# jxbi1010/VLA-Touch

Measured on AMD Instinct MI355X. Metric: refined action chunks/sec (RDT-1B chunk + DINOv2 x2 + pi_I), higher is better.
Workload: dtype bf16 model, 16-bit activations in IEEE fp16 (RDT-1B --rdt-compute f16, DINOv2 tower; same width and MFMA rate as bf16)

## Files before the change

### vla-touch_amd/csrc/vt_api.hip

```cpp
#include <string.h>
#include "vt_common.h"
#include "vt_kernels.h"
#include "vt_host.h"
#include "vt_gemm_route.h"
#include "vt_prof.h"
#include "vt_unet_int.h"
#include "../../include/vlatouch.h"

VtProfState g_vt_prof;

extern "C" {

const char* vt_last_error(void) { return vt_errbuf(); }
int vt_version(void) { return 100; }

int vt_gemm(const void* params, vt_stream_t stream) {
  if (!params) return vt_fail(VT_ERR_ARG, "vt_gemm: null params");
  const int r = vt_gemm_launch(*reinterpret_cast<const VtGemmParams*>(params), (hipStream_t)stream);
  if (r) vt_fail(r, "vt_gemm: rejected (alignment: K, lda, ldw multiples of 8 bf16 / 4 fp32; conv: cin likewise) or launch failure");
  return r;
}
int vt_gemm_route_of(const void* params) {
  if (!params) return VT_ROUTE_BAD_ARG;
  return vt_gemm_route(*reinterpret_cast<const VtGemmParams*>(params));
}
int vt_gemm_route_split(const void* params, int* head_route, int* tail_route) {
  if (!params || !head_route || !tail_route) return vt_fail(VT_ERR_ARG, "vt_gemm_route_split: null argument");
  const VtGemmParams& p = *reinterpret_cast<const VtGemmParams*>(params);
  if (vt_gemm_route(p) != VT_GEMM_ROWSPLIT) return vt_fail(VT_ERR_ARG, "vt_gemm_route_split: the block does not route to VT_ROUTE_ROWSPLIT");
  VtGemmParams head, tail;
  *head_route = vt_gemm_rowsplit(p, head, tail);
  *tail_route = vt_gemm_route(tail);
  return VT_OK;
}
int vt_tune(int knob, int value) {
  if (knob == 1 && (value == 0 || value == 4 || value == 8)) { vt_gemm_pw_tune(value); return VT_OK; }
  if (knob == 2 || knob == 8) { vt_gemm_route_tune(knob, value); return VT_OK; }
  if (knob == 4) { vt_gemm_pws_tune(value); return VT_OK; }
  if (knob == 6) { vt_attn_kvt_tune(value); return VT_OK; }
  if (knob == 7) { vt_unet_fused_tune(value); return VT_OK; }
  if (knob == 9 && (value == 0 || value == 1 || value == 3 || value == 6)) { vt_attn16g_tune(value); return VT_OK; }
  return vt_fail(VT_ERR_ARG, "vt_tune: unknown knob %d / value %d", knob, value);
}
int vt_prof_enable(int on) {
  g_vt_prof.on = on != 0;
  g_vt_prof.mode = on > 1 ? on : 1;
  if (on) { g_vt_prof.used = 0; g_vt_prof.flops = 0.0; g_vt_prof.bytes = 0.0; }
  return VT_OK;
}
int vt_prof_collect(double* total_ms, double* flops, double* bytes, long* launches) {
  double ms = 0.0;
  for (int i = 0; i < g_vt_prof.used; ++i) {
    float t = 0.f;
    if (hipEventElapsedTime(&t, g_vt_prof.ev[2 * i], g_vt_prof.ev[2 * i + 1]) != hipSuccess) return VT_ERR_LAUNCH;
    ms += t;
  }
  if (total_ms) *total_ms = ms;
  if (flops) *flops = g_vt_prof.flops;
  if (bytes) *bytes = g_vt_prof.bytes;
  if (launches) *launches = g_vt_prof.used;
  return VT_OK;
}
int vt_attention(const void* params, vt_stream_t stream) {
  if (!params) return vt_fail(VT_ERR_ARG, "vt_attention: null params");
  const int r = vt_attn_launch(*reinterpret_cast<const VtAttnParams*>(params), (hipStream_t)stream);
  if (r) vt_fail(r, "vt_attention: bad strides/sizes or launch failure");
  return r;
}
int vt_attention_kvt(const void* params, vt_stream_t stream) {
  if (!params) return vt_fail(VT_ERR_ARG, "vt_attention_kvt: null params");
  const int r = vt_attn_kvt_launch(*reinterpret_cast<const VtAttnKvtParams*>(params), (hipStream_t)stream);
  if (r) vt_fail(r, "vt_attention_kvt: bad sizes / strides (T * 64 >= B * Nk, q_rs % 8), parts without part_ws or > 16, or launch failure");
  return r;
}
size_t vt_attention_kvt_part_bytes(int B, int H, int Nq, int parts) { return vt_attn_kvt_part_bytes(B, H, Nq, parts); }
int vt_retile_kv(const void* K, const void* V, long ld, void* KV, int M, int T, int H, vt_stream_t stream) {
  if (!K || !V || !KV || M < 1 || H < 1) return vt_fail(VT_ERR_ARG, "vt_retile_kv: null source / destination or empty shape");
  const int r = vt_k_retile_kv(K, V, ld, KV, M, T, H, (hipStream_t)stream);
  if (r) vt_fail(r, "vt_retile_kv: T * 64 < M, ld % 8 or launch failure");
  return r;
}
int vt_groupnorm(const void* params, vt_stream_t stream) {
  if (!params) return vt_fail(VT_ERR_ARG, "vt_groupnorm: null params");
  const int r = vt_k_groupnorm(*reinterpret_cast<const VtGnParams*>(params), (hipStream_t)stream);
  if (r) vt_fail(r, "vt_groupnorm: unsupported group size or launch failure");
  return r;
}
int vt_rownorm(const void* x, int xdt, long ldx, void* y, int ydt, long ldy, const float* w, const float* b, int rows, int D, float eps,
               int mode, vt_stream_t stream) {
  const int r = vt_k_rownorm(x, xdt, ldx, y, ydt, ldy, w, b, rows, D, eps, mode, (hipStream_t)stream);
  if (r) vt_fail(r, "vt_rownorm: D must be a multiple of 4 and <= 2048");
  return r;
}
int vt_headnorm(void* x, int dt, long tok_stride, int heads, long tokens, const float* w, float eps, int mode, vt_stream_t stream) {
  return vt_k_headnorm(x, dt, tok_stride, heads, tokens, w, eps, mode, (hipStream_t)stream);
}
int vt_action_normalize(const float* in, float* out, const float* mins, const float* maxs, long n, int dim, float padding_factor,
                        int denormalize, vt_stream_t stream) {
  if (!in || !out || !mins || !maxs || n < 0 || dim < 1) return vt_fail(VT_ERR_ARG, "vt_action_normalize: bad argument");
  if (n == 0) return VT_OK;
  return vt_k_actnorm(in, out, mins, maxs, n, dim, padding_factor, denormalize, (hipStream_t)stream);
}

}

static_assert(VT_ROUTE_UNSUPPORTED == VT_GEMM_UNSUPPORTED && VT_ROUTE_BAD_ARG == VT_GEMM_BAD_ARG && VT_ROUTE_REG == VT_GEMM_REG && VT_ROUTE_F32R == VT_GEMM_F32R &&
              VT_ROUTE_GLDS == VT_GEMM_GLDS && VT_ROUTE_PP == VT_GEMM_PP && VT_ROUTE_PT == VT_GEMM_PT && VT_ROUTE_PPK == VT_GEMM_PPK && VT_ROUTE_PW == VT_GEMM_PW &&
              VT_ROUTE_PWS == VT_GEMM_PWS && VT_ROUTE_ROWSPLIT == VT_GEMM_ROWSPLIT, "include/vlatouch.h route codes = enum VtGemmRoute");

namespace {
template <typename T>
__global__ void mfma_selftest_kernel(float* err) {
  const int lane = threadIdx.x, g = lane >> 4, l15 = lane & 15;
  Frag<T> a, b;
  float av[8], bv[8];
  for (int j = 0; j < 8; ++j) {
    const int k = g * 8 + j;
    av[j] = (k == l15) ? 1.f : 0.f;
    bv[j] = (float)(l15 * 100 + k);
  }
  if constexpr (sizeof(T) == 2) {
    for (int j = 0; j < 8; ++j) { a.v[j] = (short)f2bf(av[j]); b.v[j] = (short)f2bf(bv[j]); }
  } else {
    for (int j = 0; j < 8; ++j) { a.v[j] = av[j]; b.v[j] = bv[j]; }
  }
  float4_t acc = {0.f, 0.f, 0.f, 0.f};
  mma16(acc, a, b);
  float e = 0.f;
  for (int r = 0; r < 4; ++r) {
    const int row = g * 4 + r, col = l15;
    float expect = (float)(col * 100 + row);
    if constexpr (sizeof(T) == 2) expect = bf2f(f2bf(expect));
    e = fmaxf(e, fabsf(acc[r] - expect));
  }
  e = wave_max(e);
  if (lane == 0) *err = e;
}
}

extern "C" int vt_selftest_mfma(float* out_err, vt_stream_t stream) {
  if (!out_err) return vt_fail(VT_ERR_ARG, "vt_selftest_mfma: null");
  hipLaunchKernelGGL((mfma_selftest_kernel<bf16_t>), dim3(1), dim3(64), 0, (hipStream_t)stream, out_err);
  hipLaunchKernelGGL((mfma_selftest_kernel<float>), dim3(1), dim3(64), 0, (hipStream_t)stream, out_err + 1);
  return vt_check_launch();
}

namespace {
__device__ __forceinline__ void philox_round(uint32_t (&c)[4], const uint32_t k0, const uint32_t k1) {
  const uint64_t p0 = (uint64_t)0xD2511F53u * c[0], p1 = (uint64_t)0xCD9E8D57u * c[2];
  const uint32_t n0 = (uint32_t)(p1 >> 32) ^ c[1] ^ k0, n1 = (uint32_t)p1, n2 = (uint32_t)(p0 >> 32) ^ c[3] ^ k1, n3 = (uint32_t)p0;
  c[0] = n0; c[1] = n1; c[2] = n2; c[3] = n3;
}
__device__ __forceinline__ void philox4x32_10(uint32_t (&c)[4], uint32_t k0, uint32_t k1) {
#pragma unroll
  for (int r = 0; r < 10; ++r) { philox_round(c, k0, k1); k0 += 0x9E3779B9u; k1 += 0xBB67AE85u; }
}
__global__ void randn_kernel(float* __restrict__ out, const long n, const unsigned long long* __restrict__ state, const int round_bf16) {
  const long q = (long)blockIdx.x * blockDim.x + threadIdx.x;
  if (q * 4 >= n) return;
  const unsigned long long key = state[0], ctr = state[1] + (unsigned long long)q;
  uint32_t c[4] = {(uint32_t)ctr, (uint32_t)(ctr >> 32), 0u, 0u};
  philox4x32_10(c, (uint32_t)key, (uint32_t)(key >> 32));
  float v[4];
#pragma unroll
  for (int h = 0; h < 2; ++h) {
    const float u1 = ((float)(c[2 * h] >> 8) + 0.5f) * (1.0f / 16777216.0f);
    const float u2 = ((float)(c[2 * h + 1] >> 8) + 0.5f) * (1.0f / 16777216.0f);
    const float r = sqrtf(-2.0f * __logf(u1));
    float sn, cs;
    __sincosf(6.283185307179586f * u2, &sn, &cs);
    v[2 * h] = r * cs; v[2 * h + 1] = r * sn;
  }
#pragma unroll
  for (int j = 0; j < 4; ++j) {
    if (round_bf16) v[j] = bf2f(f2bf(v[j]));
    if (q * 4 + j < n) out[q * 4 + j] = v[j];
  }
}
__global__ void randn_advance_kernel(unsigned long long* state, const unsigned long long by) { state[1] += by; }
template <typename TI>
__global__ void slice_cast_kernel(const TI* __restrict__ in, float* __restrict__ out, int B, int Tin, int Din, int T, int Dd) {
  const long i = (long)blockIdx.x * blockDim.x + threadIdx.x;
  if (i >= (long)B * T * Dd) return;
  const int d = (int)(i % Dd);
  const long r = i / Dd;
  const int t = (int)(r % T), b = (int)(r / T);
  out[i] = Elem<TI>::to_f(in[((long)b * Tin + t) * Din + d]);
}
}

extern "C" int vt_randn(float* out, long n, void* state, int round_bf16, vt_stream_t stream) {
  if (!out || !state || n < 0) return vt_fail(VT_ERR_ARG, "vt_randn: null argument");
  if (n == 0) return VT_OK;
  const long quads = (n + 3) / 4;
  hipLaunchKernelGGL(randn_kernel, dim3((unsigned)((quads + 255) / 256)), dim3(256), 0, (hipStream_t)stream, out, n, (const unsigned long long*)state, round_bf16);
  hipLaunchKernelGGL(randn_advance_kernel, dim3(1), dim3(1), 0, (hipStream_t)stream, (unsigned long long*)state, (unsigned long long)quads);
  return vt_check_launch();
}
extern "C" int vt_slice_cast(const void* in, int idt, float* out, int B, int Tin, int Din, int T, int Dd, vt_stream_t stream) {
  if (!in || !out || B < 1 || T < 1 || Dd < 1 || T > Tin || Dd > Din) return vt_fail(VT_ERR_ARG, "vt_slice_cast: bad shape");
  const long n = (long)B * T * Dd;
  const dim3 grid((unsigned)((n + 255) / 256));
  if (idt == VT_BF16) hipLaunchKernelGGL((slice_cast_kernel<bf16_t>), grid, dim3(256), 0, (hipStream_t)stream, (const bf16_t*)in, out, B, Tin, Din, T, Dd);
  else if (idt == VT_F32) hipLaunchKernelGGL((slice_cast_kernel<float>), grid, dim3(256), 0, (hipStream_t)stream, (const float*)in, out, B, Tin, Din, T, Dd);
  else return vt_fail(VT_ERR_UNSUPPORTED, "vt_slice_cast: bf16 or fp32 input");
  return vt_check_launch();
}

extern "C" int vt_cast(const void* in, int idt, long ldi, void* out, int odt, long ldo, int rows, int cols, vt_stream_t stream) {
  if (!in || !out || rows < 1 || cols < 1) return vt_fail(VT_ERR_ARG, "vt_cast: bad argument");
  const int r = vt_k_act_copy(in, idt, ldi, out, odt, ldo, rows, cols, VT_ACT_NONE, (hipStream_t)stream);
  if (r) vt_fail(r, "vt_cast: unsupported dtype pair");
  return r;
}
```

### vla-touch_amd/csrc/vt_gemm_pw.hip

```cpp
#include "vt_common.h"
#include "vt_gemm_route.h"
#include "vt_gemm_epilogue.h"
#include "vt_prof.h"
#include "vt_host.h"
#include "vt_kernels.h"
#include "../../include/vlatouch.h"

namespace {

constexpr int BM = 160, BN = 128, BK = 64;
constexpr int TMW = BM / 32;
constexpr int A_TILE = BM * 128;
constexpr int OPS = BM / 8 / 4 + 4;

template <typename T16, typename TC, int NB, int FUSE = 0>
__global__ __launch_bounds__(256, 1) void gemm_pw_kernel(const VtGemmParams p, const int tiles_n, const int tiles_per_group, const int total_tiles, const int GM) {
  constexpr int SMEM = NB * A_TILE > BM * BN * 4 ? NB * A_TILE : BM * BN * 4;
  __shared__ __attribute__((aligned(16))) char smem[SMEM];
  const int tid = threadIdx.x, lane = tid & 63;
  const int wave = __builtin_amdgcn_readfirstlane(tid >> 6);
  const int l31 = lane & 31, hk = lane >> 5;

  int bid = blockIdx.x;
  if ((total_tiles & 7) == 0) bid = (bid & 7) * (total_tiles >> 3) + (bid >> 3);
  const int grp = bid / tiles_per_group;
  const int t_in = bid - grp * tiles_per_group;
  const int tiles_m = tiles_per_group / tiles_n;
  const int sr = t_in / (GM * tiles_n);
  const int gmr = min(GM, tiles_m - sr * GM);
  const int r_in = t_in - sr * GM * tiles_n;
  const int tn = r_in / gmr, tm = sr * GM + (r_in - tn * gmr);
  const int m0 = tm * BM, n0 = tn * BN;

  const uint16_t* A = reinterpret_cast<const uint16_t*>(p.A) + (long)grp * p.a_gs;
  const int nk = p.K / BK;

  const __amdgpu_buffer_rsrc_t rsA = __builtin_amdgcn_make_buffer_rsrc((void*)(A + (long)m0 * p.lda), 0, 0x7fffffff, 0x00020000);
  int asrc[5];
#pragma unroll
  for (int e = 0; e < 5; ++e) {
    const int r = (wave + 4 * e) * 8 + (lane >> 3);
    const int c = (lane & 7) ^ ((r >> 1) & 7);
    asrc[e] = (int)(((long)(min(m0 + r, p.M - 1) - m0) * p.lda + c * 8) * 2);
  }
  const char* wbase = reinterpret_cast<const char*>(p.Wp) + ((long)grp * p.w_gs) * 2 + ((long)(n0 / 32 + wave) * (p.K / 16)) * 1024;
  wbase = VT_UNIFORM_PTR(wbase);
  const unsigned wvoff = lane * 16;

  int4_t wb[NB][4];
  auto issue = [&](const int kt, auto bc) {
    constexpr int b = decltype(bc)::value;
#pragma unroll
    for (int e = 0; e < 5; ++e)
      __builtin_amdgcn_raw_ptr_buffer_load_lds(rsA, (lds_void*)(smem + b * A_TILE + (wave + 4 * e) * 1024), 16, asrc[e], kt * (BK * 2), 0, 0);
    const char* sb = wbase + (long)kt * 4096;
    wload<0, true>(wb[b][0], wvoff, sb);
    wload<1024, false>(wb[b][1], wvoff, sb);
    wload<2048, false>(wb[b][2], wvoff, sb);
    wload<3072, false>(wb[b][3], wvoff, sb);
  };

  const int xr = (l31 >> 1) & 7;
  int foff[4];
#pragma unroll
  for (int s = 0; s < 4; ++s) foff[s] = l31 * 128 + (((s * 2 + hk) ^ xr) * 16);
  auto frags = [&](int4_t (&f)[TMW], const int b, const int s) {
#pragma unroll
    for (int j = 0; j < TMW; ++j) f[j] = *reinterpret_cast<const int4_t*>(smem + b * A_TILE + j * 4096 + foff[s]);
  };

  float16_t acc[TMW];
#pragma unroll
  for (int j = 0; j < TMW; ++j)
#pragma unroll
    for (int r = 0; r < 16; ++r) acc[j][r] = 0.f;

  static_for<NB - 1>([&](auto bc) { if (decltype(bc)::value < nk) issue(decltype(bc)::value, bc); });
  vt_wait_vm<(NB - 3) * OPS>(wb[0]);
  vt_wait_vm<(NB - 3) * OPS>(wb[1]);
  __builtin_amdgcn_sched_barrier(0);
  __builtin_amdgcn_s_barrier();
  __builtin_amdgcn_sched_barrier(0);
  int4_t af[2][TMW];
  frags(af[0], 0, 0);

  constexpr int RSV = FUSE == 2 ? (BM * 16 + 255) / 256 : 1;
  float4 rsv[RSV];
  auto sub = [&](const int t, auto uc, auto tailc) {
    constexpr int U = decltype(uc)::value;
    constexpr bool TAIL = decltype(tailc)::value;
    if constexpr (!TAIL || U == 0) issue(t + NB - 1, std::integral_constant<int, (U + NB - 1) % NB>{});
    if constexpr (FUSE == 2 && TAIL && U == NB - 2) {
      const int h2 = p.rs_n >> 1, nq = BM * h2;
#pragma unroll
      for (int i = 0; i < RSV; ++i) {
        const int q = tid + 256 * i;
        const int row = q / h2, c = q - row * h2;
        rsv[i] = q < nq ? *reinterpret_cast<const float4*>(p.rs_part + ((long)min(m0 + row, p.M - 1) * p.rs_n + 2 * c) * 2) : make_float4(0.f, 0.f, 0.f, 0.f);
      }
    }
#pragma unroll
    for (int s = 0; s < 4; ++s) {
      if (s < 3) frags(af[(s + 1) & 1], U, s + 1);
      else if (!TAIL || U < NB - 1) frags(af[0], (U + 1) % NB, 0);
#pragma unroll
      for (int j = 0; j < TMW; ++j) acc[j] = mma32<T16>(wb[U][s], af[s & 1][j], acc[j]);
    }
#pragma unroll
    for (int i = 0; i < 4 * TMW; ++i) {
      __builtin_amdgcn_sched_group_barrier(0x008, 1, 0);
      __builtin_amdgcn_sched_group_barrier(0x100, 1, 0);
    }
    if constexpr (!TAIL) vt_wait_vm<(NB - 3) * OPS>(wb[(U + 2) % NB]);
    else if constexpr (U + 2 < NB) vt_wait_vm<(NB - 3 - U > 0 ? NB - 3 - U : 0) * OPS>(wb[(U + 2) % NB]);
    __builtin_amdgcn_sched_barrier(0);
    __builtin_amdgcn_s_barrier();
    __builtin_amdgcn_sched_barrier(0);
  };
  int t = 0;
  for (; t + NB < nk; t += NB) static_for<NB>([&](auto uc) { sub(t + decltype(uc)::value, uc, std::false_type{}); });
  static_for<NB>([&](auto uc) { sub(t + decltype(uc)::value, uc, std::true_type{}); });

  float* tile = reinterpret_cast<float*>(smem);
  float rs[TMW];
#pragma unroll
  for (int j = 0; j < TMW; ++j) rs[j] = 1.f;
  if constexpr (FUSE == 2) {
    float2* pair = reinterpret_cast<float2*>(tile + BM);
    const int h2 = p.rs_n >> 1;
#pragma unroll
    for (int i = 0; i < RSV; ++i) {
      const int q = tid + 256 * i;
      if (q < BM * h2) {
        const float dS = rsv[i].y - rsv[i].w;
        pair[q] = make_float2(rsv[i].x + rsv[i].z + (p.rs_mode == 2 ? dS * dS * (1.0f / 128.0f) : 0.f), rsv[i].y + rsv[i].w);
      }
    }
    __syncthreads();
    if (tid < BM) {
      float var;
      if (p.rs_mode == 2) {
        float na = 0.f, mean = 0.f, m2 = 0.f;
        for (int c = 0; c < h2; ++c) {
          const float2 v = pair[tid * h2 + c];
          const float delta = v.y * (1.0f / 128.0f) - mean, nt = na + 128.0f;
          mean += delta * (128.0f / nt);
          m2 += v.x + delta * delta * (na * 128.0f / nt);
          na = nt;
        }
        var = m2 / (1.0f / p.rs_inv_k - 1.0f);
      } else {
        float sq = 0.f;
        for (int c = 0; c < h2; ++c) sq += pair[tid * h2 + c].x;
        var = sq * p.rs_inv_k;
      }
      tile[tid] = rsqrtf(var + p.rs_eps);
    }
    __syncthreads();
#pragma unroll
    for (int j = 0; j < TMW; ++j) rs[j] = tile[j * 32 + l31];
    __syncthreads();
  }
  const int half = wave & 1, c4 = lane & 15;
  const int ncol0 = n0 + half * 64, n = ncol0 + c4 * 4;
  const bool col_ok = n < p.N;
  const int rbase = (wave >> 1) * (BM / 2) + (lane >> 4);
  TC* Cg = reinterpret_cast<TC*>(p.C) + (long)grp * p.c_gs;
  const TC* Rg = p.residual ? reinterpret_cast<const TC*>(p.residual) + (long)grp * p.r_gs : nullptr;
  constexpr bool PRE = sizeof(TC) == 4;
  float4 rpre[PRE ? BM / 8 : 1];
  const bool use_pre = PRE && Rg != nullptr;
  if constexpr (PRE) {
    if (use_pre) {
#pragma unroll
      for (int it = 0; it < BM / 8; ++it) {
        const int m = min(m0 + rbase + it * 4, p.M - 1);
        rpre[it] = col_ok ? *reinterpret_cast<const float4*>(reinterpret_cast<const float*>(Rg) + (long)m * p.ldr + n) : make_float4(0.f, 0.f, 0.f, 0.f);
      }
    }
  }
  const float* bias = p.bias ? p.bias + (long)grp * p.bias_gs : nullptr;
  const float* hw = nullptr;
  if (p.hn_w0 && ncol0 < p.hn_c0_end) hw = p.hn_w0;
  else if (p.hn_w1 && ncol0 >= p.hn_c0_end && ncol0 < p.hn_c1_end) hw = p.hn_w1;
  const float4 zero4 = make_float4(0.f, 0.f, 0.f, 0.f), one4 = make_float4(1.f, 1.f, 1.f, 1.f);
  const float4 b4 = (bias && col_ok) ? *reinterpret_cast<const float4*>(bias + n) : zero4;
  const float4 cs4 = (p.colscale && col_ok) ? *reinterpret_cast<const float4*>(p.colscale + n) : one4;
  const float4 hw4 = hw ? *reinterpret_cast<const float4*>(hw + c4 * 4) : one4;
  float4 g4 = zero4;
  if constexpr (FUSE == 1) { if (col_ok && p.xn_gain) g4 = *reinterpret_cast<const float4*>(p.xn_gain + n); }
  __builtin_amdgcn_sched_barrier(0);
  constexpr int PFN = 8;
  unsigned pfv[PFN];
#pragma unroll
  for (int i = 0; i < PFN; ++i) pfv[i] = 0;
  if (p.pf_ptr) {
    const unsigned nbytes = (unsigned)p.pf_bytes;
    const unsigned share = ((nbytes + (unsigned)total_tiles - 1u) / (unsigned)total_tiles + 63u) & ~63u;
    const unsigned b0 = blockIdx.x * share;
    const __amdgpu_buffer_rsrc_t rsP = __builtin_amdgcn_make_buffer_rsrc((void*)((const char*)p.pf_ptr + b0), 0,
                                                                        b0 < nbytes ? (int)min(share, nbytes - b0) : 0, 0x00020000);
#pragma unroll
    for (int i = 0; i < PFN; ++i)
      if ((unsigned)i * 16384u < share) pfv[i] = __builtin_amdgcn_raw_buffer_load_b32(rsP, (i * 256 + tid) * 64, 0, 0);
  }
  __builtin_amdgcn_sched_barrier(0);
#pragma unroll
  for (int j = 0; j < TMW; ++j) {
    const int m = j * 32 + l31;
    const float r = FUSE == 2 ? rs[j] : 1.f;
#pragma unroll
    for (int rq = 0; rq < 4; ++rq) {
      const int n4 = wave * 8 + rq * 2 + hk;
      *reinterpret_cast<float4*>(tile + m * BN + ((n4 ^ (m & 7)) * 4)) =
          make_float4(acc[j][rq * 4] * r, acc[j][rq * 4 + 1] * r, acc[j][rq * 4 + 2] * r, acc[j][rq * 4 + 3] * r);
    }
  }
  __syncthreads();
  if (p.act != VT_ACT_NONE) {
#pragma unroll 2
    for (int it = 0; it < BM / 8; ++it) {
      const int row = rbase + it * 4;
      const float4 x = *reinterpret_cast<const float4*>(tile + row * BN + (((half * 16 + c4) ^ (row & 7)) * 4));
      vt_epi_segment<TC, 0, true>(p, x, b4, cs4, hw, hw4, Cg, Rg, m0 + row, n, ncol0, col_ok);
    }
  } else if (FUSE == 1 && PRE && use_pre) {
    if constexpr (PRE && FUSE == 1) {
      T16* Xn = reinterpret_cast<T16*>(p.xn_out);
      const int pcol = 2 * tn + half, pn = 2 * tiles_n;
#pragma unroll
      for (int it = 0; it < BM / 8; ++it) {
        const int row = rbase + it * 4, m = m0 + row;
        const float4 x = *reinterpret_cast<const float4*>(tile + row * BN + (((half * 16 + c4) ^ (row & 7)) * 4));
        float o[4] = {x.x + b4.x, x.y + b4.y, x.z + b4.z, x.w + b4.w};
        o[0] *= cs4.x; o[1] *= cs4.y; o[2] *= cs4.z; o[3] *= cs4.w;
        o[0] += rpre[it].x; o[1] += rpre[it].y; o[2] += rpre[it].z; o[3] += rpre[it].w;
        const bool ok = m < p.M && col_ok;
        const float q1 = row16_sum(ok ? (o[0] + o[1]) + (o[2] + o[3]) : 0.f);
        float q;
        if (p.rs_mode == 2) {
          const float mj = q1 * (1.0f / 64.0f);
          const float d0 = o[0] - mj, d1 = o[1] - mj, d2 = o[2] - mj, d3 = o[3] - mj;
          q = row16_sum(ok ? (d0 * d0 + d1 * d1) + (d2 * d2 + d3 * d3) : 0.f);
        } else q = row16_sum(ok ? (o[0] * o[0] + o[1] * o[1]) + (o[2] * o[2] + o[3] * o[3]) : 0.f);
        if (ok) {
          vt_epi_st128(reinterpret_cast<float*>(Cg) + (long)m * p.ldc + n, make_float4(o[0], o[1], o[2], o[3]));
          constexpr float LIM = std::is_same<T16, half_t>::value ? 65504.0f : 3.0e38f;
          auto sat = [](float v) { return fminf(fmaxf(v, -LIM), LIM); };
          const float xg[4] = {o[0] * g4.x, o[1] * g4.y, o[2] * g4.z, o[3] * g4.w};
          if constexpr (std::is_same<T16, half_t>::value) {
            if (fmaxf(fmaxf(fabsf(xg[0]), fabsf(xg[1])), fmaxf(fabsf(xg[2]), fabsf(xg[3]))) > LIM) vt_range_note(p.range_flag, VT_RANGE_XN_SAT);
          }
          T16 ov[4] = {Elem<T16>::from_f(sat(xg[0])), Elem<T16>::from_f(sat(xg[1])), Elem<T16>::from_f(sat(xg[2])), Elem<T16>::from_f(sat(xg[3]))};
          vt_epi_st64(Xn + (long)m * p.xn_ld + n, *reinterpret_cast<const uint2*>(ov));
        }
        if (c4 == 0 && m < p.M) *reinterpret_cast<float2*>(p.xn_part + ((long)m * pn + pcol) * 2) = make_float2(q, q1);
      }
    }
  } else if (use_pre) {
#pragma unroll
    for (int it = 0; it < BM / 8; ++it) {
      const int row = rbase + it * 4;
      const float4 x = *reinterpret_cast<const float4*>(tile + row * BN + (((half * 16 + c4) ^ (row & 7)) * 4));
      vt_epi_segment<TC, 0, false>(p, x, b4, cs4, hw, hw4, Cg, nullptr, m0 + row, n, ncol0, col_ok, &rpre[PRE ? it : 0]);
    }
  } else {
#pragma unroll 4
    for (int it = 0; it < BM / 8; ++it) {
      const int row = rbase + it * 4;
      const float4 x = *reinterpret_cast<const float4*>(tile + row * BN + (((half * 16 + c4) ^ (row & 7)) * 4));
      vt_epi_segment<TC, 0, false>(p, x, b4, cs4, hw, hw4, Cg, Rg, m0 + row, n, ncol0, col_ok);
    }
  }
#pragma unroll
  for (int i = 0; i < PFN; ++i) asm volatile("" :: "v"(pfv[i]));
}

__global__ void pack_w32_kernel(const uint16_t* __restrict__ W, const long ldw, uint16_t* __restrict__ out, const int N, const int K) {
  const long i = (long)blockIdx.x * blockDim.x + threadIdx.x;
  const long nchunks = (long)N * K / 8;
  if (i >= nchunks) return;
  const int lane = (int)(i & 63);
  const long frag = i >> 6;
  const int ks = (int)(frag % (K / 16));
  const int nt = (int)(frag / (K / 16));
  const int n = nt * 32 + (lane & 31), k = ks * 16 + (lane >> 5) * 8;
  *reinterpret_cast<uint4*>(out + i * 8) = *reinterpret_cast<const uint4*>(W + (long)n * ldw + k);
}

}

static int g_vt_pw_nb = 0;

void vt_gemm_pw_tune(int ring) { g_vt_pw_nb = ring; }

bool vt_gemm_pw_fits(const VtGemmParams& p) {
  if (!p.Wp || p.cmap || p.groups != 1) return false;
  if (p.N % BN || p.K % (8 * BK) || p.lda >= (1 << 21)) return false;
  const long tiles = (long)((p.M + BM - 1) / BM) * (p.N / BN) * p.groups;
  const long rounds = (tiles + 255) / 256;
  return tiles >= 100 && tiles * 8 >= rounds * 256 * 7;
}

int vt_gemm_pw_launch(const VtGemmParams& p, hipStream_t s) {
  const int tiles_n = p.N / BN, tiles_m = (p.M + BM - 1) / BM;
  const int per_group = tiles_n * tiles_m, total = per_group * p.groups;
  const int gm = 4;
  VtProfScope prof(3, p, s);
  const bool c16 = p.c_dtype != VT_F32;
#define VT_PW_GO(T16, TC) do { if (g_vt_pw_nb == 8) hipLaunchKernelGGL((gemm_pw_kernel<T16, TC, 8>), dim3(total), dim3(256), 0, s, p, tiles_n, per_group, total, gm); \
                               else hipLaunchKernelGGL((gemm_pw_kernel<T16, TC, 4>), dim3(total), dim3(256), 0, s, p, tiles_n, per_group, total, gm); } while (0)
  if (p.xn_out || p.rs_part) {
    const dim3 g(total), b(256);
    if (p.xn_out && (c16 || !p.residual || p.act != VT_ACT_NONE || p.hn_w0 || p.hn_w1)) return VT_ERR_UNSUPPORTED;
    if (p.xn_out && p.rs_part) return VT_ERR_UNSUPPORTED;
    if (p.xn_out) {
      if (p.a_dtype == VT_BF16) hipLaunchKernelGGL((gemm_pw_kernel<bf16_t, float, 4, 1>), g, b, 0, s, p, tiles_n, per_group, total, gm);
      else hipLaunchKernelGGL((gemm_pw_kernel<half_t, float, 4, 1>), g, b, 0, s, p, tiles_n, per_group, total, gm);
    } else if (!c16) {
      return VT_ERR_UNSUPPORTED;
    } else if (p.a_dtype == VT_BF16) {
      hipLaunchKernelGGL((gemm_pw_kernel<bf16_t, bf16_t, 4, 2>), g, b, 0, s, p, tiles_n, per_group, total, gm);
    } else {
      hipLaunchKernelGGL((gemm_pw_kernel<half_t, half_t, 4, 2>), g, b, 0, s, p, tiles_n, per_group, total, gm);
    }
    return vt_check_launch();
  }
  if (p.a_dtype == VT_BF16) { if (c16) VT_PW_GO(bf16_t, bf16_t); else VT_PW_GO(bf16_t, float); }
  else { if (c16) VT_PW_GO(half_t, half_t); else VT_PW_GO(half_t, float); }
#undef VT_PW_GO
  return vt_check_launch();
}

extern "C" int vt_pack_w32(const void* W, long ldw, void* out, int N, int K, vt_stream_t stream) {
  if (!W || !out || N <= 0 || K <= 0 || N % 32 || K % 16 || ldw % 8) return vt_fail(VT_ERR_ARG, "vt_pack_w32: N %% 32, K %% 16, ldw %% 8 must be 0");
  const long nchunks = (long)N * K / 8;
  hipLaunchKernelGGL(pack_w32_kernel, dim3((unsigned)((nchunks + 255) / 256)), dim3(256), 0, (hipStream_t)stream, (const uint16_t*)W, ldw, (uint16_t*)out, N, K);
  return vt_check_launch();
}
```

### vla-touch_amd/csrc/vt_gemm_route.h

```cpp
#pragma once
#include <hip/hip_runtime.h>
#include "vt_gemm.h"

enum VtGemmRoute : int {
  VT_GEMM_UNSUPPORTED = 0,
  VT_GEMM_BAD_ARG = 1,
  VT_GEMM_REG = 2,
  VT_GEMM_F32R = 3,
  VT_GEMM_GLDS = 4,
  VT_GEMM_PP = 5,
  VT_GEMM_PT = 6,
  VT_GEMM_PPK = 7,
  VT_GEMM_PW = 8,
  VT_GEMM_PWS = 9,
  VT_GEMM_ROWSPLIT = 10,
};

VtGemmRoute vt_gemm_route(const VtGemmParams& p);
VtGemmRoute vt_gemm_rowsplit(const VtGemmParams& p, VtGemmParams& head, VtGemmParams& tail);
void vt_gemm_route_tune(int knob, int value);

bool vt_gemm_lds_fits(const VtGemmParams& p);
bool vt_gemm_can_fuse_headnorm(const VtGemmParams& p);
bool vt_gemm_pp_fits(const VtGemmParams& p);
bool vt_gemm_pt_fits(const VtGemmParams& p);
bool vt_gemm_pt_one_round(const VtGemmParams& p);
bool vt_gemm_ppk_fits(const VtGemmParams& p);
bool vt_gemm_pw_fits(const VtGemmParams& p);
bool vt_gemm_pws_fits(const VtGemmParams& p);
bool vt_gemm_f32r_fits(const VtGemmParams& p);

int vt_gemm_reg_launch(const VtGemmParams& p, hipStream_t s);
int vt_gemm_f32r_launch(const VtGemmParams& p, hipStream_t s);
int vt_gemm_fast_launch(const VtGemmParams& p, hipStream_t s);
int vt_gemm_pp_launch(const VtGemmParams& p, hipStream_t s);
int vt_gemm_pt_launch(const VtGemmParams& p, hipStream_t s);
int vt_gemm_ppk_launch(const VtGemmParams& p, hipStream_t s);
int vt_gemm_pw_launch(const VtGemmParams& p, hipStream_t s);
int vt_gemm_pws_launch(const VtGemmParams& p, hipStream_t s);
void vt_gemm_pw_tune(int ring);
void vt_gemm_pws_tune(int split);
```

Measured before the change: 402.6.

## Add dedicated loader wave for A-tile LDS fills in packed-weight GEMM

```diff
diff --git a/vla-touch_amd/csrc/vt_api.hip b/vla-touch_amd/csrc/vt_api.hip
--- a/vla-touch_amd/csrc/vt_api.hip
+++ b/vla-touch_amd/csrc/vt_api.hip
@@ -37,6 +37,7 @@
   if (knob == 1 && (value == 0 || value == 4 || value == 8)) { vt_gemm_pw_tune(value); return VT_OK; }
   if (knob == 2 || knob == 8) { vt_gemm_route_tune(knob, value); return VT_OK; }
   if (knob == 4) { vt_gemm_pws_tune(value); return VT_OK; }
+  if (knob == 10) { vt_gemm_pw_loader_tune(value); return VT_OK; }
   if (knob == 6) { vt_attn_kvt_tune(value); return VT_OK; }
   if (knob == 7) { vt_unet_fused_tune(value); return VT_OK; }
   if (knob == 9 && (value == 0 || value == 1 || value == 3 || value == 6)) { vt_attn16g_tune(value); return VT_OK; }
diff --git a/vla-touch_amd/csrc/vt_gemm_pw.hip b/vla-touch_amd/csrc/vt_gemm_pw.hip
--- a/vla-touch_amd/csrc/vt_gemm_pw.hip
+++ b/vla-touch_amd/csrc/vt_gemm_pw.hip
@@ -13,13 +13,19 @@
 constexpr int A_TILE = BM * 128;
 constexpr int OPS = BM / 8 / 4 + 4;
 
-template <typename T16, typename TC, int NB, int FUSE = 0>
-__global__ __launch_bounds__(256, 1) void gemm_pw_kernel(const VtGemmParams p, const int tiles_n, const int tiles_per_group, const int total_tiles, const int GM) {
+__device__ __forceinline__ int lane_now() {
+  int l;
+  asm volatile("v_mbcnt_lo_u32_b32 %0, -1, 0\n\tv_mbcnt_hi_u32_b32 %0, -1, %0" : "=v"(l));
+  return l;
+}
+
+template <typename T16, typename TC, int NB, int FUSE = 0, bool LW = false>
+__global__ __launch_bounds__(LW ? 320 : 256, LW ? 3 : 1) void gemm_pw_kernel(const VtGemmParams p, const int tiles_n, const int tiles_per_group, const int total_tiles, const int GM) {
   constexpr int SMEM = NB * A_TILE > BM * BN * 4 ? NB * A_TILE : BM * BN * 4;
   __shared__ __attribute__((aligned(16))) char smem[SMEM];
-  const int tid = threadIdx.x, lane = tid & 63;
+  int tid = threadIdx.x, lane = tid & 63;
   const int wave = __builtin_amdgcn_readfirstlane(tid >> 6);
-  const int l31 = lane & 31, hk = lane >> 5;
+  int l31 = lane & 31, hk = lane >> 5;
 
   int bid = blockIdx.x;
   if ((total_tiles & 7) == 0) bid = (bid & 7) * (total_tiles >> 3) + (bid >> 3);
@@ -35,6 +41,52 @@
   const uint16_t* A = reinterpret_cast<const uint16_t*>(p.A) + (long)grp * p.a_gs;
   const int nk = p.K / BK;
 
+  if constexpr (LW) {
+    static_assert(NB == 4, "the loader wave's counted waits are written for the 4-deep ring");
+    if (wave == 4) {
+      constexpr int PCS = BM / 8;
+      const __amdgpu_buffer_rsrc_t rsL = __builtin_amdgcn_make_buffer_rsrc((void*)(A + (long)m0 * p.lda), 0, 0x7fffffff, 0x00020000);
+      const int ll = lane_now();
+      int lsrc[PCS];
+#pragma unroll
+      for (int q = 0; q < PCS; ++q) {
+        const int r = q * 8 + (ll >> 3);
+        const int c = (ll & 7) ^ ((r >> 1) & 7);
+        lsrc[q] = (int)(((long)(min(m0 + r, p.M - 1) - m0) * p.lda + c * 8) * 2);
+      }
+      auto fill = [&](const int kt, auto bc) {
+        constexpr int b = decltype(bc)::value;
+#pragma unroll
+        for (int q = 0; q < PCS; ++q)
+          __builtin_amdgcn_raw_ptr_buffer_load_lds(rsL, (lds_void*)(smem + b * A_TILE + q * 1024), 16, lsrc[q], kt * (BK * 2), 0, 0);
+      };
+      auto hand = [&](auto nc) {
+        if constexpr (decltype(nc)::value >= 0) vt_wait_vm<decltype(nc)::value * PCS>();
+        __builtin_amdgcn_sched_barrier(0);
+        __builtin_amdgcn_s_barrier();
+        __builtin_amdgcn_sched_barrier(0);
+      };
+      static_for<NB - 1>([&](auto bc) { fill(decltype(bc)::value, bc); });
+      hand(std::integral_constant<int, NB - 3>{});
+      int t = 0;
+      for (; t + NB < nk; t += NB)
+        static_for<NB>([&](auto uc) {
+          constexpr int U = decltype(uc)::value;
+          fill(t + U + NB - 1, std::integral_constant<int, (U + NB - 1) % NB>{});
+          hand(std::integral_constant<int, NB - 3>{});
+        });
+      static_for<NB>([&](auto uc) {
+        constexpr int U = decltype(uc)::value;
+        if constexpr (U == 0) fill(t + NB - 1, std::integral_constant<int, NB - 1>{});
+        hand(std::integral_constant<int, (U + 2 < NB) ? (NB - 3 - U > 0 ? NB - 3 - U : 0) : -1>{});
+      });
+#pragma unroll
+      for (int i = 0; i < (FUSE == 2 ? 4 : 1); ++i) __builtin_amdgcn_s_barrier();
+      return;
+    }
+  }
+  constexpr int WOPS = LW ? 4 : OPS;
+
   const __amdgpu_buffer_rsrc_t rsA = __builtin_amdgcn_make_buffer_rsrc((void*)(A + (long)m0 * p.lda), 0, 0x7fffffff, 0x00020000);
   int asrc[5];
 #pragma unroll
@@ -50,15 +102,21 @@
   int4_t wb[NB][4];
   auto issue = [&](const int kt, auto bc) {
     constexpr int b = decltype(bc)::value;
-#pragma unroll
-    for (int e = 0; e < 5; ++e)
-      __builtin_amdgcn_raw_ptr_buffer_load_lds(rsA, (lds_void*)(smem + b * A_TILE + (wave + 4 * e) * 1024), 16, asrc[e], kt * (BK * 2), 0, 0);
+    if constexpr (!LW) {
+#pragma unroll
+      for (int e = 0; e < 5; ++e)
+        __builtin_amdgcn_raw_ptr_buffer_load_lds(rsA, (lds_void*)(smem + b * A_TILE + (wave + 4 * e) * 1024), 16, asrc[e], kt * (BK * 2), 0, 0);
+    }
     const char* sb = wbase + (long)kt * 4096;
     wload<0, true>(wb[b][0], wvoff, sb);
     wload<1024, false>(wb[b][1], wvoff, sb);
     wload<2048, false>(wb[b][2], wvoff, sb);
     wload<3072, false>(wb[b][3], wvoff, sb);
   };
+  auto issue_w = [&](const int kt, auto bc, auto sc) {
+    constexpr int b = decltype(bc)::value, s = decltype(sc)::value;
+    wload<s * 1024, s == 0>(wb[b][s], wvoff, wbase + (long)kt * 4096);
+  };
 
   const int xr = (l31 >> 1) & 7;
   int foff[4];
@@ -76,8 +134,8 @@
     for (int r = 0; r < 16; ++r) acc[j][r] = 0.f;
 
   static_for<NB - 1>([&](auto bc) { if (decltype(bc)::value < nk) issue(decltype(bc)::value, bc); });
-  vt_wait_vm<(NB - 3) * OPS>(wb[0]);
-  vt_wait_vm<(NB - 3) * OPS>(wb[1]);
+  vt_wait_vm<(NB - 3) * WOPS>(wb[0]);
+  vt_wait_vm<(NB - 3) * WOPS>(wb[1]);
   __builtin_amdgcn_sched_barrier(0);
   __builtin_amdgcn_s_barrier();
   __builtin_amdgcn_sched_barrier(0);
@@ -89,30 +147,34 @@
   auto sub = [&](const int t, auto uc, auto tailc) {
     constexpr int U = decltype(uc)::value;
     constexpr bool TAIL = decltype(tailc)::value;
-    if constexpr (!TAIL || U == 0) issue(t + NB - 1, std::integral_constant<int, (U + NB - 1) % NB>{});
-    if constexpr (FUSE == 2 && TAIL && U == NB - 2) {
+    constexpr bool ISSUES = !TAIL || U == 0;
+    if constexpr (ISSUES && !LW) issue(t + NB - 1, std::integral_constant<int, (U + NB - 1) % NB>{});
+    if constexpr (FUSE == 2 && TAIL && (U == NB - 2 || (LW && U == NB - 1))) {
       const int h2 = p.rs_n >> 1, nq = BM * h2;
-#pragma unroll
-      for (int i = 0; i < RSV; ++i) {
-        const int q = tid + 256 * i;
+      const int tq = LW ? wave * 64 + lane_now() : tid;
+      constexpr int I0 = LW && U == NB - 1 ? RSV / 2 : 0, I1 = LW && U == NB - 2 ? RSV / 2 : RSV;
+#pragma unroll
+      for (int i = I0; i < I1; ++i) {
+        const int q = tq + 256 * i;
         const int row = q / h2, c = q - row * h2;
         rsv[i] = q < nq ? *reinterpret_cast<const float4*>(p.rs_part + ((long)min(m0 + row, p.M - 1) * p.rs_n + 2 * c) * 2) : make_float4(0.f, 0.f, 0.f, 0.f);
       }
     }
-#pragma unroll
-    for (int s = 0; s < 4; ++s) {
-      if (s < 3) frags(af[(s + 1) & 1], U, s + 1);
-      else if (!TAIL || U < NB - 1) frags(af[0], (U + 1) % NB, 0);
+    static_for<4>([&](auto sc) {
+      constexpr int s = decltype(sc)::value;
+      if constexpr (s < 3) frags(af[(s + 1) & 1], U, s + 1);
+      else if constexpr (!TAIL || U < NB - 1) frags(af[0], (U + 1) % NB, 0);
 #pragma unroll
       for (int j = 0; j < TMW; ++j) acc[j] = mma32<T16>(wb[U][s], af[s & 1][j], acc[j]);
-    }
+      if constexpr (ISSUES && LW) issue_w(t + NB - 1, std::integral_constant<int, (U + NB - 1) % NB>{}, sc);
+    });
 #pragma unroll
     for (int i = 0; i < 4 * TMW; ++i) {
       __builtin_amdgcn_sched_group_barrier(0x008, 1, 0);
       __builtin_amdgcn_sched_group_barrier(0x100, 1, 0);
     }
-    if constexpr (!TAIL) vt_wait_vm<(NB - 3) * OPS>(wb[(U + 2) % NB]);
-    else if constexpr (U + 2 < NB) vt_wait_vm<(NB - 3 - U > 0 ? NB - 3 - U : 0) * OPS>(wb[(U + 2) % NB]);
+    if constexpr (!TAIL) vt_wait_vm<(NB - 3) * WOPS>(wb[(U + 2) % NB]);
+    else if constexpr (U + 2 < NB) vt_wait_vm<(NB - 3 - U > 0 ? NB - 3 - U : 0) * WOPS>(wb[(U + 2) % NB]);
     __builtin_amdgcn_sched_barrier(0);
     __builtin_amdgcn_s_barrier();
     __builtin_amdgcn_sched_barrier(0);
@@ -120,6 +182,7 @@
   int t = 0;
   for (; t + NB < nk; t += NB) static_for<NB>([&](auto uc) { sub(t + decltype(uc)::value, uc, std::false_type{}); });
   static_for<NB>([&](auto uc) { sub(t + decltype(uc)::value, uc, std::true_type{}); });
+  if constexpr (LW) { lane = lane_now(); tid = wave * 64 + lane; l31 = lane & 31; hk = lane >> 5; }
 
   float* tile = reinterpret_cast<float*>(smem);
   float rs[TMW];
@@ -170,10 +233,11 @@
   constexpr bool PRE = sizeof(TC) == 4;
   float4 rpre[PRE ? BM / 8 : 1];
   const bool use_pre = PRE && Rg != nullptr;
+  constexpr int RH = LW ? BM / 16 : BM / 8;
   if constexpr (PRE) {
     if (use_pre) {
 #pragma unroll
-      for (int it = 0; it < BM / 8; ++it) {
+      for (int it = 0; it < RH; ++it) {
         const int m = min(m0 + rbase + it * 4, p.M - 1);
         rpre[it] = col_ok ? *reinterpret_cast<const float4*>(reinterpret_cast<const float*>(Rg) + (long)m * p.ldr + n) : make_float4(0.f, 0.f, 0.f, 0.f);
       }
@@ -217,6 +281,15 @@
     }
   }
   __syncthreads();
+  if constexpr (PRE && LW) {
+    if (use_pre) {
+#pragma unroll
+      for (int it = RH; it < BM / 8; ++it) {
+        const int m = min(m0 + rbase + it * 4, p.M - 1);
+        rpre[it] = col_ok ? *reinterpret_cast<const float4*>(reinterpret_cast<const float*>(Rg) + (long)m * p.ldr + n) : make_float4(0.f, 0.f, 0.f, 0.f);
+      }
+    }
+  }
   if (p.act != VT_ACT_NONE) {
 #pragma unroll 2
     for (int it = 0; it < BM / 8; ++it) {
@@ -291,8 +364,10 @@
 }
 
 static int g_vt_pw_nb = 0;
+static int g_vt_pw_lw = 1;
 
 void vt_gemm_pw_tune(int ring) { g_vt_pw_nb = ring; }
+void vt_gemm_pw_loader_tune(int on) { g_vt_pw_lw = on != 0; }
 
 bool vt_gemm_pw_fits(const VtGemmParams& p) {
   if (!p.Wp || p.cmap || p.groups != 1) return false;
@@ -308,27 +383,29 @@
   const int gm = 4;
   VtProfScope prof(3, p, s);
   const bool c16 = p.c_dtype != VT_F32;
-#define VT_PW_GO(T16, TC) do { if (g_vt_pw_nb == 8) hipLaunchKernelGGL((gemm_pw_kernel<T16, TC, 8>), dim3(total), dim3(256), 0, s, p, tiles_n, per_group, total, gm); \
-                               else hipLaunchKernelGGL((gemm_pw_kernel<T16, TC, 4>), dim3(total), dim3(256), 0, s, p, tiles_n, per_group, total, gm); } while (0)
+  const bool lw = g_vt_pw_lw != 0;
+#define VT_PW_RUN(T16, TC, NB, FUSE) do { if (lw && NB == 4) hipLaunchKernelGGL((gemm_pw_kernel<T16, TC, 4, FUSE, true>), dim3(total), dim3(320), 0, s, p, tiles_n, per_group, total, gm); \
+                                          else hipLaunchKernelGGL((gemm_pw_kernel<T16, TC, NB, FUSE, false>), dim3(total), dim3(256), 0, s, p, tiles_n, per_group, total, gm); } while (0)
+#define VT_PW_GO(T16, TC) do { if (g_vt_pw_nb == 8) VT_PW_RUN(T16, TC, 8, 0); else VT_PW_RUN(T16, TC, 4, 0); } while (0)
   if (p.xn_out || p.rs_part) {
-    const dim3 g(total), b(256);
     if (p.xn_out && (c16 || !p.residual || p.act != VT_ACT_NONE || p.hn_w0 || p.hn_w1)) return VT_ERR_UNSUPPORTED;
     if (p.xn_out && p.rs_part) return VT_ERR_UNSUPPORTED;
     if (p.xn_out) {
-      if (p.a_dtype == VT_BF16) hipLaunchKernelGGL((gemm_pw_kernel<bf16_t, float, 4, 1>), g, b, 0, s, p, tiles_n, per_group, total, gm);
-      else hipLaunchKernelGGL((gemm_pw_kernel<half_t, float, 4, 1>), g, b, 0, s, p, tiles_n, per_group, total, gm);
+      if (p.a_dtype == VT_BF16) VT_PW_RUN(bf16_t, float, 4, 1);
+      else VT_PW_RUN(half_t, float, 4, 1);
     } else if (!c16) {
       return VT_ERR_UNSUPPORTED;
     } else if (p.a_dtype == VT_BF16) {
-      hipLaunchKernelGGL((gemm_pw_kernel<bf16_t, bf16_t, 4, 2>), g, b, 0, s, p, tiles_n, per_group, total, gm);
+      VT_PW_RUN(bf16_t, bf16_t, 4, 2);
     } else {
-      hipLaunchKernelGGL((gemm_pw_kernel<half_t, half_t, 4, 2>), g, b, 0, s, p, tiles_n, per_group, total, gm);
+      VT_PW_RUN(half_t, half_t, 4, 2);
     }
     return vt_check_launch();
   }
   if (p.a_dtype == VT_BF16) { if (c16) VT_PW_GO(bf16_t, bf16_t); else VT_PW_GO(bf16_t, float); }
   else { if (c16) VT_PW_GO(half_t, half_t); else VT_PW_GO(half_t, float); }
 #undef VT_PW_GO
+#undef VT_PW_RUN
   return vt_check_launch();
 }
 
diff --git a/vla-touch_amd/csrc/vt_gemm_route.h b/vla-touch_amd/csrc/vt_gemm_route.h
--- a/vla-touch_amd/csrc/vt_gemm_route.h
+++ b/vla-touch_amd/csrc/vt_gemm_route.h
@@ -39,4 +39,5 @@
 int vt_gemm_pw_launch(const VtGemmParams& p, hipStream_t s);
 int vt_gemm_pws_launch(const VtGemmParams& p, hipStream_t s);
 void vt_gemm_pw_tune(int ring);
+void vt_gemm_pw_loader_tune(int on);
 void vt_gemm_pws_tune(int split);
```

Result: no change. 404.3 (median of 6 runs) (+0.4%).
